# mahaarbo/casclik

Measured on AMD Instinct MI355X. Metric: CLIK steps/sec (whole node), 7-DoF 3-task priority stack, batch 16384, higher is better.
Workload: dtype f64

## Files before the change

casclik_amd/csrc/clik_pinv_team.hpp:

```cpp
#pragma once
#include "clik_pinv_static.hpp"

namespace clik {


constexpr int TEAM_WAVES = 4;
constexpr int TEAM_INST = TEAM_WAVES * WAVE / TEAM;

template <int CTRL>
__device__ __forceinline__ double quad_perm_f64(const double x)
{
    int lo = __double2loint(x), hi = __double2hiint(x);
    lo = __builtin_amdgcn_mov_dpp(lo, CTRL, 0xf, 0xf, true);
    hi = __builtin_amdgcn_mov_dpp(hi, CTRL, 0xf, 0xf, true);
    return __hiloint2double(hi, lo);
}
constexpr int QUAD_LANE0 = 0x00;

template <const ShapeDesc& SD>
inline size_t team_lds_bytes(bool values = false)
{
    if (values) return 0;
    return ((size_t)StaticLayout<SD>::IMG_DOUBLES + (size_t)(SD.n + (SD.n_y > 0 ? SD.n_y : 0)) * TEAM_INST) * sizeof(double);
}

#ifndef CLIK_RESIDENT_PIPELINE
#define CLIK_RESIDENT_PIPELINE 1
#endif

struct RoleConsts {
    double beta, hsel, nsolo, cax, cx2, lam0, kap, hp;
};
__device__ __forceinline__ RoleConsts role_consts_computed(const int r, const double lam)
{
    const double one_lam = 1.0 + lam;
    const bool hi = (r & 2) != 0, solo = (r == 0) || (r == 3);
    RoleConsts rc;
    rc.beta = (r == 1) ? 0.5 * lam : ((r == 2) ? one_lam : lam);
    rc.hsel = solo ? 1.0 : 0.0;
    rc.nsolo = solo ? 0.0 : 1.0;
    rc.cax = hi ? one_lam : 1.0;
    rc.cx2 = hi ? 1.0 : 0.0;
    rc.lam0 = (r == 0) ? lam : 0.0;
    rc.kap = hi ? 1.0 / one_lam : 1.0;
    rc.hp = hi ? 1.0 : 0.0;
    return rc;
}
struct RoleTable {
    double v[TEAM][8];
};
constexpr RoleTable role_table(const double lam)
{
    const double one_lam = 1.0 + lam;
    return RoleTable{{{lam, 1.0, 0.0, 1.0, 0.0, lam, 1.0, 0.0},
                      {0.5 * lam, 0.0, 1.0, 1.0, 0.0, 0.0, 1.0, 0.0},
                      {one_lam, 0.0, 1.0, one_lam, 1.0, 0.0, 1.0 / one_lam, 1.0},
                      {lam, 1.0, 0.0, one_lam, 1.0, 0.0, 1.0 / one_lam, 1.0}}};
}
template <class IMGV>
inline __constant__ RoleTable kRoleTable = role_table(IMGV::value.lam);
#ifndef CLIK_ROLE_TABLE
#define CLIK_ROLE_TABLE 1
#endif
template <class IMGV>
__device__ __forceinline__ RoleConsts role_consts_loaded(const int r)
{
#if !CLIK_ROLE_TABLE
    return role_consts_computed(r, IMGV::value.lam);
#endif
    typedef double d2 __attribute__((ext_vector_type(2)));
    const d2* p = reinterpret_cast<const d2*>(&kRoleTable<IMGV>.v[r][0]);
    const d2 a = p[0], b = p[1], c = p[2], d = p[3];
    return RoleConsts{a.x, a.y, b.x, b.y, c.x, c.y, d.x, d.y};
}

struct NoMidTick {
    __device__ __forceinline__ void operator()(const double) const {}
};
template <const ShapeDesc& SD, class MID = NoMidTick>
__device__ __forceinline__ void team_tick(const Img<SD>* __restrict__ Slds, const TickArgs& tk,
                                          const double (&z)[SD.n], const double* ysl, const double a0, const double a1,
                                          const int r, const int inst, const RoleConsts& rc, const SinCosK& sck,
                                          double (&v)[SD.n], bool& in_tc, MID&& mid = MID())
{
    constexpr int N = SD.n, M = SD.m[1], M0 = SD.m[0], M2 = SD.m[2];
    constexpr int NT = M * (M + 1) / 2;
    TaskCache<SD> tc;
    CLIK_PHASE("sincos");
    {
        double sns[N], css[N];
        if constexpr (SD.uses_fk != 0) {
            double sn0, cs0, sn1, cs1;
            sincos_fast(a0, sn0, cs0, sck);
            sincos_fast(a1, sn1, cs1, sck);
            const bool huge = (fabs(a0) > kSinCosFastMax) | (fabs(a1) > kSinCosFastMax);
            if (__builtin_expect(__ballot(huge) != 0ull, 0)) {
                if (fabs(a0) > kSinCosFastMax) { const SinCos sc = sincos_slow(a0); sn0 = sc.s; cs0 = sc.c; }
                if (fabs(a1) > kSinCosFastMax) { const SinCos sc = sincos_slow(a1); sn1 = sc.s; cs1 = sc.c; }
            }
            CLIK_PHASE("sincos_exchange");
            static_for<0, N>([&](auto jc) __attribute__((always_inline)) {
                constexpr int j = decltype(jc)::value;
                if constexpr (shape_state_type(SD, j) == CLIK_JOINT_REVOLUTE) {
                    constexpr int CTRL = (j / 2) * 0x55;
                    sns[j] = quad_perm_f64<CTRL>((j & 1) ? sn1 : sn0);
                    css[j] = quad_perm_f64<CTRL>((j & 1) ? cs1 : cs0);
                } else {
                    sns[j] = css[j] = 0.0;
                }
            });
        }
        const Img<SD> Sfk = *Slds;
        __builtin_amdgcn_sched_barrier(0);
        CLIK_PHASE("fk");
        Kin<N> K;
        if constexpr (SD.uses_fk != 0) {
            forward_kinematics_sc<SD>(&Sfk, z, sns, css, K);
            if constexpr (SD.quat_src != 0) orientation_feature_s<SD>(&Sfk, ysl, inst, K);
        }
        CLIK_PHASE("task_rows");
        cache_task<SD, 0>(&Sfk, tk, K, z, ysl, inst, tc);
    }

    const Img<SD> Sb = *Slds;
    __builtin_amdgcn_sched_barrier(0);
    CLIK_PHASE("desired");
    const Img<SD>* __restrict__ S = &Sb;
    const double lam = S->lam;
    const double one_lam = 1.0 + lam;

    double des1[M], w2[N];
    {
        double e[M], Jt[M], ke[M];
        task_values<SD, 1>(S, tk, tc, z, ysl, inst, e, Jt);
        gain_apply_s<M, SD.gain_matrix[1] != 0>(S->tasks[1], e, ke);
#pragma unroll
        for (int i = 0; i < M; ++i) des1[i] = SD.feedforward != 0 ? -ke[i] - Jt[i] : -ke[i];
    }
    {
        double e[M2], Jt[M2], ke[M2];
        task_values<SD, 2>(S, tk, tc, z, ysl, inst, e, Jt);
        gain_apply_s<M2, SD.gain_matrix[2] != 0>(S->tasks[2], e, ke);
#pragma unroll
        for (int j = 0; j < N; ++j) w2[j] = 0.0;
        const double* Pm = S->cpinv[2];
        static_for<0, M2>([&](auto ic) __attribute__((always_inline)) {
            constexpr int i = decltype(ic)::value;
            constexpr int col = SD.ucol[2][i] - 1;
            const double d = SD.feedforward != 0 ? -ke[i] - Jt[i] : -ke[i];
            w2[col] = Pm[col * CLIK_MAX_M + i] * d;
        });
    }
    double e0[M0], Jt0[M0];
    task_values<SD, 0>(S, tk, tc, z, ysl, inst, e0, Jt0);
    double sact[N], p0[N];
    static_for<0, M0>([&](auto ic) __attribute__((always_inline)) {
        constexpr int i = decltype(ic)::value;
        constexpr int col = SD.ucol[0][i] - 1;
        sact[col] = ((e0[i] - S->tasks[0].set_max[i] > 0.0) | (e0[i] - S->tasks[0].set_min[i] < 0.0)) ? 1.0 : 0.0;
        p0[col] = S->cpinv[0][col * CLIK_MAX_M + i];
    });

    CLIK_PHASE("gram");
    double Gm[NT];
#pragma unroll
    for (int i = 0; i < M; ++i)
#pragma unroll
        for (int k = 0; k <= i; ++k) {
            double acc = 0.0;
#pragma unroll
            for (int j = 0; j < N; ++j) acc = fma(jac<SD, 1>(S, tc, i, j), jac<SD, 1>(S, tc, k, j), acc);
            Gm[tri(i, k)] = acc;
        }

    if constexpr (!std::is_same<std::decay_t<MID>, NoMidTick>::value) {
        mid(Gm[0]);
    }
    CLIK_PHASE("role_rhs");
    double X[N], rhs[M];
#pragma unroll
    for (int j = 0; j < N; ++j) X[j] = w2[j] * fma(-rc.cx2, sact[j], rc.cax);
#pragma unroll
    for (int i = 0; i < M; ++i) {
        double sacc = 0.0;
#pragma unroll
        for (int j = 0; j < N; ++j) sacc = fma(jac<SD, 1>(S, tc, i, j), X[j], sacc);
        rhs[i] = fma(rc.nsolo, sacc, rc.hsel * des1[i]);
    }
    double A[NT], rd[M], s2[M];
#pragma unroll
    for (int i = 0; i < M; ++i)
#pragma unroll
        for (int k = 0; k <= i; ++k) A[tri(i, k)] = (i == k) ? Gm[tri(i, k)] + rc.beta : Gm[tri(i, k)];
    CLIK_PHASE("factor");
    ldl_factor_s<M>(A, rd);
    CLIK_PHASE("solve1");
    ldl_solve_s<M>(A, rd, rhs);
    CLIK_PHASE("solve2");
#pragma unroll
    for (int i = 0; i < M; ++i) s2[i] = rhs[i];
    ldl_solve_s<M>(A, rd, s2);
#pragma unroll
    for (int i = 0; i < M; ++i) rhs[i] = fma(rc.lam0, s2[i], rhs[i]);
    CLIK_PHASE("jt_product");
    double g[N];
#pragma unroll
    for (int j = 0; j < N; ++j) {
        double sacc = 0.0;
#pragma unroll
        for (int i = 0; i < M; ++i) sacc = fma(jac<SD, 1>(S, tc, i, j), rhs[i], sacc);
        g[j] = sacc;
    }

    
    CLIK_PHASE("meet");
#pragma unroll
    for (int j = 0; j < N; ++j) {
        const double other = quad_perm_f64<0xB1>(g[j]);
        const double nmul = fma(-p0[j] * rc.hp, sact[j], 1.0);
        v[j] = fma(g[j], nmul, rc.kap * (X[j] - other));
    }
    CLIK_PHASE("cone");
    {
        const clik_task& t = S->tasks[0];
        double le[M0], ue[M0];
#pragma unroll
        for (int i = 0; i < M0; ++i) {
            le[i] = e0[i] - t.set_min[i];
            ue[i] = e0[i] - t.set_max[i];
        }
        double le_min = le[0], ue_max = ue[0];
#pragma unroll
        for (int i = 1; i < M0; ++i) {
            le_min = fmin(le_min, le[i]);
            ue_max = fmax(ue_max, ue[i]);
        }
        const bool outside = (le_min < 1e-12) | (ue_max > 1e-12);
        in_tc = true;
        if (__builtin_amdgcn_ballot_w64(outside) != 0ull) {
            double od = 0.0, nde = 0.0, nout = 0.0, ndiff = 0.0;
            static_for<0, M0>([&](auto ic) __attribute__((always_inline)) {
                constexpr int i = decltype(ic)::value;
                constexpr int col = SD.ucol[0][i] - 1;
                const double de = Jt0[i] + v[col];
                const double hl = half_sign(le[i]), hu = half_sign(ue[i]);
                ndiff += fabs(hl - hu);
                const double out = hl + hu;
                od = fma(out, de, od);
                nde = fma(de, de, nde);
                nout = fma(out, out, nout);
            });
            const bool corner = ndiff == 0.0;
            bool going_in = od < 0.0;
            if (__builtin_amdgcn_ballot_w64(corner & outside) != 0ull) {
                const double dists = (sqrt(nde) + 1e-10) * sqrt(nout);
                const bool steep = (od < 0.0) & (fabs(od) / dists < 0.70710678118654757);
                going_in = corner ? steep : going_in;
            }
            in_tc = !outside | going_in;
        }
    }
    CLIK_PHASE_END();
}

template <int K>
struct RawImage {
    unsigned long long w[K];
};

template <const ShapeDesc& SD, class IMGV = void>
__global__ __launch_bounds__(TEAM_WAVES * WAVE) void pinv_solve_static_team_kernel(
    const void* __restrict__ img_g, const double* __restrict__ q, const double* __restrict__ y,
    double* __restrict__ dq, int32_t* __restrict__ mode_out, const long long B, const TickArgs tk)
{
    static_assert(shape_team_ok(SD), "shape outside the team kernel's family");
    constexpr bool VALUES = !std::is_void<IMGV>::value;
    extern __shared__ double lds[];
    constexpr int N = SD.n, M = SD.m[1], M0 = SD.m[0], M2 = SD.m[2], NY = SD.n_y > 0 ? SD.n_y : 0;
    constexpr int NT = M * (M + 1) / 2;
    constexpr int NTHREADS = TEAM_WAVES * WAVE;
    const int tid = threadIdx.x;
    const int wave = __builtin_amdgcn_readfirstlane(tid >> 6);
    const int r = tid & (TEAM - 1);
    const int inst = tid >> 2;
    const long long b0 = (long long)blockIdx.x * TEAM_INST;
    const long long left = B - b0;
    const int rows_valid = left < TEAM_INST ? (int)left : TEAM_INST;
    double* zs = lds + (VALUES ? 0 : StaticLayout<SD>::IMG_DOUBLES);
    double* ys = zs + N * TEAM_INST;
    typedef double d2 __attribute__((ext_vector_type(2)));
    CLIK_STAMP_W(0, 0);
    CLIK_BODY_BEGIN();
    CLIK_PHASE("rows_in");
    const unsigned uinst = (unsigned)blockIdx.x * (unsigned)TEAM_INST + (unsigned)inst;
    const unsigned ulast = (unsigned)B - 1u;
    const unsigned urow = uinst < ulast ? uinst : ulast;
    const long long binst = (long long)urow;
    double zdir[N], ydir[NY > 0 ? NY : 1];
    RoleConsts rc;
    const int j0 = 2 * r < N ? 2 * r : N - 1, j1 = 2 * r + 1 < N ? 2 * r + 1 : N - 1;
    double a0 = 0.0, a1 = 0.0;
    const SinCosK sck = sincos_consts();
    __builtin_amdgcn_sched_barrier(0);
    if constexpr (VALUES) {
        const unsigned qoff = __umul24(urow, (unsigned)(N * sizeof(double)));
        a0 = *reinterpret_cast<const double*>(reinterpret_cast<const char*>(q) + (qoff + (unsigned)j0 * 8u));
        a1 = *reinterpret_cast<const double*>(reinterpret_cast<const char*>(q) + (qoff + (unsigned)j1 * 8u));
        __builtin_amdgcn_sched_barrier(0);
        const double* __restrict__ qrow = reinterpret_cast<const double*>(reinterpret_cast<const char*>(q) + qoff);
#pragma unroll
        for (int j = 0; j < N; ++j) zdir[j] = qrow[j];
        __builtin_amdgcn_sched_barrier(0);
        if constexpr (NY > 0) {
            const double* __restrict__ yrow = reinterpret_cast<const double*>(reinterpret_cast<const char*>(y) + __umul24(urow, (unsigned)(NY * sizeof(double))));
#pragma unroll
            for (int k = 0; k < NY; ++k) ydir[k] = yrow[k];
        }
        __builtin_amdgcn_sched_barrier(0);
        rc = role_consts_loaded<IMGV>(r);
        __builtin_amdgcn_sched_barrier(0);
    }
    if constexpr (!VALUES) {
        constexpr int CH = VALUES ? 0 : StaticLayout<SD>::IMG_CHUNKS;
        constexpr int PER = VALUES ? 1 : (CH + TEAM_WAVES - 1) / TEAM_WAVES;
        constexpr int QR = (N * TEAM_INST + NTHREADS - 1) / NTHREADS;
        constexpr int YR = (NY * TEAM_INST + NTHREADS - 1) / NTHREADS;
        const d2* src = (const d2*)img_g;
        d2* dst = (d2*)lds;
        const int lane = tid & (WAVE - 1);
        d2 img[PER];
        if constexpr (!VALUES) {
#pragma unroll
            for (int k = 0; k < PER; ++k) {
                const int ck = k * TEAM_WAVES + wave;
                img[k] = src[(ck < CH ? ck : CH - 1) * WAVE + lane];
            }
        }
        double qv[QR], yv[YR > 0 ? YR : 1];
        const double* qg = q + b0 * N;
        const int qlast = rows_valid * N - 1;
#pragma unroll
        for (int i = 0; i < QR; ++i) {
            const int k = i * NTHREADS + tid;
            qv[i] = qg[k < qlast ? k : qlast];
        }
        if constexpr (NY > 0) {
            const double* yg = y + b0 * NY;
            const int ylast = rows_valid * NY - 1;
#pragma unroll
            for (int i = 0; i < YR; ++i) {
                const int k = i * NTHREADS + tid;
                yv[i] = yg[k < ylast ? k : ylast];
            }
        }
        if constexpr (!VALUES) {
#pragma unroll
            for (int k = 0; k < PER; ++k) {
                const int ck = k * TEAM_WAVES + wave;
                if (ck < CH) dst[ck * WAVE + lane] = img[k];
            }
        }
#pragma unroll
        for (int i = 0; i < QR; ++i) {
            const int k = i * NTHREADS + tid;
            if (k < N * TEAM_INST) zs[k] = qv[i];
        }
        if constexpr (NY > 0) {
#pragma unroll
            for (int i = 0; i < YR; ++i) {
                const int k = i * NTHREADS + tid;
                if (k < NY * TEAM_INST) ys[k] = yv[i];
            }
        }
        __syncthreads();
    }
    CLIK_STAMP_W(0, 1);
    constexpr Img<SD> Sval = []() constexpr { if constexpr (VALUES) return IMGV::value; else return Img<SD>{}; }();
    const Img<SD>* __restrict__ Slds = VALUES ? &Sval : (const Img<SD>*)lds;
    const double* ysl = VALUES ? ydir : ys + inst * NY;
    if constexpr (!VALUES) rc = role_consts_computed(r, Slds->lam);
    double z[N];
#pragma unroll
    for (int j = 0; j < N; ++j) z[j] = VALUES ? zdir[j] : zs[inst * N + j];

    if constexpr (!VALUES) {
        a0 = zs[inst * N + j0];
        a1 = zs[inst * N + j1];
    }
    double v[N];
    bool in_tc;
    team_tick<SD>(Slds, tk, z, ysl, a0, a1, r, inst, rc, sck, v, in_tc);
    CLIK_STAMP_W(0, 6);
    CLIK_PHASE("select_store");
    const bool ok0 = __builtin_amdgcn_mov_dpp((int)in_tc, QUAD_LANE0, 0xf, 0xf, true) != 0;
    if constexpr (VALUES) {
        if (r == (ok0 ? 0 : 3) && uinst <= ulast) {
            double* __restrict__ drow = reinterpret_cast<double*>(reinterpret_cast<char*>(dq) + __umul24(uinst, (unsigned)(N * sizeof(double))));
#pragma unroll
            for (int j = 0; j < N; ++j) drow[j] = v[j];
            if (mode_out != nullptr)
                *reinterpret_cast<int32_t*>(reinterpret_cast<char*>(mode_out) + uinst * 4u) = ok0 ? 0 : 1;
        }
    } else {
        if (r == (ok0 ? 0 : 3)) {
#pragma unroll
            for (int j = 0; j < N; ++j) zs[inst * N + j] = v[j];
            if (mode_out != nullptr && inst < rows_valid) mode_out[b0 + inst] = ok0 ? 0 : 1;
        }
        __syncthreads();
        constexpr int QR = (N * TEAM_INST + NTHREADS - 1) / NTHREADS;
        double* dg = dq + b0 * N;
        const int total = rows_valid * N;
#pragma unroll
        for (int i = 0; i < QR; ++i) {
            const int k = i * NTHREADS + tid;
            if (k < total) dg[k] = zs[k];
        }
    }
    CLIK_STAMP_W(0, 5);
    CLIK_BODY_END();
    CLIK_PHASE_END();
}

template <const ShapeDesc& SD, class IMGV = void, int STAGES = 1>
__global__ __launch_bounds__(TEAM_WAVES * WAVE) void pinv_rollout_static_team_kernel(
    const void* __restrict__ img_g, double* __restrict__ q, const double* __restrict__ y,
    double* __restrict__ dq, int32_t* __restrict__ mode_out, const long long B,
    const double* __restrict__ tterms, const int n_ticks, const double dt, const double max_speed)
{
    static_assert(STAGES == 1 || STAGES == 4, "explicit Euler or classical Runge-Kutta");
    constexpr int stages = STAGES;
    static_assert(shape_team_ok(SD), "shape outside the team kernel's family");
    constexpr bool VALUES = !std::is_void<IMGV>::value;
    extern __shared__ double lds[];
    constexpr int N = SD.n, NY = SD.n_y > 0 ? SD.n_y : 0;
    const int tid = threadIdx.x;
    const int wave = __builtin_amdgcn_readfirstlane(tid >> 6);
    const int r = tid & (TEAM - 1);
    const int inst = tid >> 2;
    const long long b0 = (long long)blockIdx.x * TEAM_INST;
    const bool valid = b0 + inst < B;
    const long long binst = valid ? (b0 + inst) : (B - 1);
    double* ys = lds + (VALUES ? 0 : StaticLayout<SD>::IMG_DOUBLES);
    double z[N], ydir[NY > 0 ? NY : 1];
#pragma unroll
    for (int j = 0; j < N; ++j) z[j] = q[binst * N + j];
    if constexpr (NY > 0) {
#pragma unroll
        for (int k = 0; k < NY; ++k) ydir[k] = y[binst * NY + k];
    }
    if constexpr (!VALUES) {
        typedef double d2 __attribute__((ext_vector_type(2)));
        constexpr int CH = StaticLayout<SD>::IMG_CHUNKS;
        const d2* src = (const d2*)img_g;
        d2* dst = (d2*)lds;
        const int lane = tid & (WAVE - 1);
        for (int ck = wave; ck < CH; ck += TEAM_WAVES) dst[ck * WAVE + lane] = src[ck * WAVE + lane];
        if constexpr (NY > 0) {
#pragma unroll
            for (int k = 0; k < NY; ++k) ys[inst * NY + k] = ydir[k];
        }
        __syncthreads();
    }
    constexpr Img<SD> Sval = []() constexpr { if constexpr (VALUES) return IMGV::value; else return Img<SD>{}; }();
    const Img<SD>* __restrict__ Slds = VALUES ? &Sval : (const Img<SD>*)lds;
    const double* ysl = VALUES ? ydir : ys + inst * NY;
    RoleConsts rc;
    if constexpr (VALUES) rc = role_consts_loaded<IMGV>(r);
    else rc = role_consts_computed(r, Slds->lam);
    const SinCosK sck = sincos_consts();
    const int nts = Slds->n_tslots;
    double vout[N];
    int acc_mode = -1;
#pragma unroll
    for (int j = 0; j < N; ++j) vout[j] = 0.0;
    const double vmax = max_speed > 0.0 ? max_speed : 1.7976931348623157e308;
    auto accepted = [&](const double (&v)[N], const bool ok0, double (&d)[N]) __attribute__((always_inline)) {
#pragma unroll
        for (int j = 0; j < N; ++j) d[j] = quad_perm_f64<0x00>(v[j]);
        if (__builtin_amdgcn_ballot_w64(!ok0) != 0ull) {
            if (!ok0) {
#pragma unroll
                for (int j = 0; j < N; ++j) d[j] = quad_perm_f64<0xFF>(v[j]);
            }
        }
#pragma unroll
        for (int j = 0; j < N; ++j) d[j] = fmax(fmin(d[j], vmax), -vmax);
    };
    auto sincos_args = [&](const double (&zz)[N], double& a0, double& a1) __attribute__((always_inline)) {
        a0 = zz[N - 1];
        a1 = zz[N - 1];
        static_for<0, TEAM>([&](auto kc) __attribute__((always_inline)) {
            constexpr int k = decltype(kc)::value;
            if constexpr (2 * k < N) a0 = (r == k) ? zz[2 * k] : a0;
            if constexpr (2 * k + 1 < N) a1 = (r == k) ? zz[2 * k + 1] : a1;
        });
    };
#pragma unroll 1
    for (int tick = 0; tick < n_ticks; ++tick) {
        if constexpr (STAGES == 1) {
            asm volatile("" ::: "memory");
            const TickArgs& tk = *reinterpret_cast<const TickArgs*>(tterms + (size_t)tick * 2 * nts);
            double a0, a1;
            sincos_args(z, a0, a1);
            double v[N];
            bool in_tc;
            team_tick<SD>(Slds, tk, z, ysl, a0, a1, r, inst, rc, sck, v, in_tc);
            const bool ok0 = __builtin_amdgcn_mov_dpp((int)in_tc, QUAD_LANE0, 0xf, 0xf, true) != 0;
            accepted(v, ok0, vout);
#pragma unroll
            for (int j = 0; j < N; ++j) z[j] = fma(vout[j], dt, z[j]);
            acc_mode = ok0 ? 0 : 1;
        } else {
        double z0[N], ks[N];
        int mode0 = -1;
#pragma unroll
        for (int j = 0; j < N; ++j) {
            z0[j] = z[j];
            ks[j] = 0.0;
        }
#pragma unroll 1
        for (int st = 0; st < stages; ++st) {
            asm volatile("" ::: "memory");
            const TickArgs& tk = *reinterpret_cast<const TickArgs*>(tterms + ((size_t)tick * stages + st) * 2 * nts);
            double a0, a1;
            sincos_args(z, a0, a1);
            double v[N], d[N];
            bool in_tc;
            team_tick<SD>(Slds, tk, z, ysl, a0, a1, r, inst, rc, sck, v, in_tc);
            const bool ok0 = __builtin_amdgcn_mov_dpp((int)in_tc, QUAD_LANE0, 0xf, 0xf, true) != 0;
            accepted(v, ok0, d);
            const double wgt = (st == 0 || st == 3) ? 1.0 : 2.0;
            const double cnext = (st == 2) ? dt : 0.5 * dt;
#pragma unroll
            for (int j = 0; j < N; ++j) {
                ks[j] = fma(wgt, d[j], ks[j]);
                z[j] = fma(d[j], cnext, z0[j]);
            }
            mode0 = (st == 0) ? (ok0 ? 0 : 1) : mode0;
        }
#pragma unroll
        for (int j = 0; j < N; ++j) {
            vout[j] = ks[j] * (1.0 / 6.0);
            z[j] = fma(vout[j], dt, z0[j]);
        }
        acc_mode = mode0;
        }
    }
    if (r == 0 && valid) {
#pragma unroll
        for (int j = 0; j < N; ++j) {
            q[(b0 + inst) * N + j] = z[j];
            dq[(b0 + inst) * N + j] = vout[j];
        }
        if (mode_out != nullptr) mode_out[b0 + inst] = acc_mode;
    }
}

struct ResidentTicket {
    unsigned in_seq, p0[15];
    unsigned ring_depth, p1a;
    double integrate_dt, max_speed;
    unsigned p1[10];
    unsigned stop, p2[15];
    unsigned waves, ticks_done, p3[14];
};
static_assert(sizeof(ResidentTicket) == 256, "clik_ticket layout (include/clik.h)");

__device__ __forceinline__ unsigned long long realtime_100mhz()
{
    unsigned long long t;
    asm volatile("s_memrealtime %0\n\ts_waitcnt lgkmcnt(0)" : "=s"(t)::"memory");
    return t;
}

template <int NE>
struct RowStage {
    static constexpr int BLOCK = 16 * NE * 8;
    static constexpr int PIECES = (BLOCK + 1023) / 1024;
    static constexpr int DOUBLES = NE > 0 ? PIECES * 128 : 0;
};
template <int NE>
__device__ __forceinline__ int stage_rows(const double* base, const long long row0, const long long total_rows,
                                          double* lds, const int lane, const bool al16)
{
    constexpr int BLOCK = RowStage<NE>::BLOCK;
    long long r0 = row0 < total_rows - 16 ? row0 : total_rows - 16;
    r0 = r0 > 0 ? r0 : 0;
    const char* src = reinterpret_cast<const char*>(base) + r0 * (NE * 8);
    const long long room = (total_rows - r0) * (NE * 8);
    if (al16 && room >= 16) {
#pragma unroll
        for (int p = 0; p < RowStage<NE>::PIECES; ++p) {
            int off = p * 1024 + lane * 16;
            off = off < BLOCK - 16 ? off : BLOCK - 16;
            off = off < room - 16 ? off : (int)(room - 16);
            __builtin_amdgcn_global_load_lds((const __attribute__((address_space(1))) void*)(src + off),
                                             (__attribute__((address_space(3))) void*)(lds + p * 128), 16, 0, 17);
        }
    } else {
#pragma unroll
        for (int p = 0; p < 4 * RowStage<NE>::PIECES; ++p) {
            int off = p * 256 + lane * 4;
            off = off < BLOCK - 4 ? off : BLOCK - 4;
            off = off < room - 4 ? off : (int)(room - 4);
            __builtin_amdgcn_global_load_lds((const __attribute__((address_space(1))) void*)(src + off),
                                             (__attribute__((address_space(3))) void*)(lds + p * 32), 4, 0, 17);
        }
    }
    return (int)(row0 - r0);
}
__device__ __forceinline__ int stage_row(const int i, const int shift) { return (i + shift) < 15 ? (i + shift) : 15; }

struct ResidentWave {
    ResidentTicket* ticket;
    unsigned* done;
    unsigned long long polls, max_polls;
    unsigned seen, slot;
    bool leave, lane0, first;

    __device__ __forceinline__ void init(ResidentTicket* t, unsigned* d, const unsigned long long budget, const int n_ticks,
                                         const unsigned wave_slot, const unsigned n_waves, const int tid)
    {
        ticket = t;
        done = d;
        polls = 0;
        max_polls = budget;
        seen = 0u;
        slot = wave_slot;
        leave = false;
        lane0 = (tid & (WAVE - 1)) == 0;
        first = wave_slot == 0u && tid == 0;
        if (first) {
            ticket->waves = n_waves;
            ticket->p3[0] = (unsigned)budget;
            ticket->p3[1] = (unsigned)(budget >> 32);
            ticket->p3[2] = (unsigned)n_ticks;
        }
    }
    __device__ __forceinline__ void poll_for(const unsigned want)
    {
#pragma unroll 1
        for (;;) {
            seen = __hip_atomic_load(&ticket->in_seq, __ATOMIC_RELAXED, __HIP_MEMORY_SCOPE_SYSTEM);
            if (seen >= want) {
                __atomic_signal_fence(__ATOMIC_ACQUIRE);
                return;
            }
            if (__hip_atomic_load(&ticket->stop, __ATOMIC_RELAXED, __HIP_MEMORY_SCOPE_SYSTEM) != 0u) {
                leave = true;
                return;
            }
            if (++polls > max_polls) {
                __hip_atomic_store(&ticket->stop, 2u, __ATOMIC_RELAXED, __HIP_MEMORY_SCOPE_SYSTEM);
                if (lane0) {
                    ticket->p3[3] = (unsigned)polls;
                    ticket->p3[4] = slot;
                }
                leave = true;
                return;
            }
            __builtin_amdgcn_s_sleep(1);
        }
    }
    __device__ __forceinline__ void peek() { seen = __hip_atomic_load(&ticket->in_seq, __ATOMIC_RELAXED, __HIP_MEMORY_SCOPE_SYSTEM); }
    __device__ __forceinline__ unsigned look() const { return __hip_atomic_load(&ticket->in_seq, __ATOMIC_RELAXED, __HIP_MEMORY_SCOPE_SYSTEM); }
    __device__ __forceinline__ void publish_done(const int k)
    {
        asm volatile("s_waitcnt vmcnt(0)" ::: "memory");
        if (lane0) __hip_atomic_store(done + slot, (unsigned)k, __ATOMIC_RELAXED, __HIP_MEMORY_SCOPE_SYSTEM);
        if (first) ticket->ticks_done = (unsigned)k;
    }
    __device__ __forceinline__ long long ring_depth() const
    {
        const unsigned raw = __hip_atomic_load(&ticket->ring_depth, __ATOMIC_RELAXED, __HIP_MEMORY_SCOPE_SYSTEM);
        return raw > 1u ? (long long)raw : 1ll;
    }
};

template <const ShapeDesc& SD, class IMGV, bool INTEGRATE = false>
__global__ __launch_bounds__(TEAM_WAVES * WAVE) void pinv_resident_team_kernel(
    const double* q, const double* y, double* dq, int32_t* mode_out, const long long B, const TickArgs tk,
    ResidentTicket* ticket, unsigned* done, const int n_ticks, const unsigned long long max_polls)
{
    static_assert(shape_team_ok(SD), "shape outside the team kernel's family");
    static_assert(!std::is_void<IMGV>::value, "resident ticks: value-specialised instantiation only");
    constexpr int N = SD.n, NY = SD.n_y > 0 ? SD.n_y : 0;
    const int tid = threadIdx.x;
    const int r = tid & (TEAM - 1);
    const int inst = tid >> 2;
    const long long b0 = (long long)blockIdx.x * TEAM_INST;
    const bool valid = b0 + inst < B;
    const long long binst = valid ? (b0 + inst) : (B - 1);
    constexpr Img<SD> Sval = IMGV::value;
    CLIK_PHASE("res_setup");
    const RoleConsts rc = role_consts_loaded<IMGV>(r);
    const SinCosK sck = sincos_consts();
    unsigned long long polls = 0;
    if (blockIdx.x == 0 && tid == 0) {
        ticket->waves = gridDim.x * TEAM_WAVES;
        ticket->p3[0] = (unsigned)max_polls;
        ticket->p3[1] = (unsigned)(max_polls >> 32);
        ticket->p3[2] = (unsigned)n_ticks;
    }
    double zn[N], yn[NY > 0 ? NY : 1];
    bool have_next = false, leave = false;
    unsigned seen = 0u;
    auto poll_for = [&](const unsigned want) __attribute__((always_inline)) {
#pragma unroll 1
        for (;;) {
            seen = __hip_atomic_load(&ticket->in_seq, __ATOMIC_RELAXED, __HIP_MEMORY_SCOPE_SYSTEM);
            if (seen >= want) {
                __atomic_signal_fence(__ATOMIC_ACQUIRE);
                return;
            }
            if (__hip_atomic_load(&ticket->stop, __ATOMIC_RELAXED, __HIP_MEMORY_SCOPE_SYSTEM) != 0u) {
                leave = true;
                return;
            }
            if (++polls > max_polls) {
                __hip_atomic_store(&ticket->stop, 2u, __ATOMIC_RELAXED, __HIP_MEMORY_SCOPE_SYSTEM);
                if ((tid & (WAVE - 1)) == 0) {
                    ticket->p3[3] = (unsigned)polls;
                    ticket->p3[4] = blockIdx.x * TEAM_WAVES + (tid >> 6);
                }
                leave = true;
                return;
            }
            __builtin_amdgcn_s_sleep(1);
        }
    };
    const unsigned ring_raw = __hip_atomic_load(&ticket->ring_depth, __ATOMIC_RELAXED, __HIP_MEMORY_SCOPE_SYSTEM);
    const long long ring = ring_raw > 1u ? (long long)ring_raw : 1ll;
    const double step_dt = INTEGRATE ? ticket->integrate_dt : 0.0, step_clamp = INTEGRATE ? ticket->max_speed : 0.0;
    constexpr bool integrate = INTEGRATE;
    double zstate[INTEGRATE ? N : 1];
#pragma unroll
    for (int j = 0; j < (INTEGRATE ? N : 1); ++j) zstate[j] = 0.0;
    constexpr int RQ = (N + 2 * TEAM - 1) / (2 * TEAM);
    using SQ = RowStage<N>;
    using SY = RowStage<NY>;
    __shared__ double stage[TEAM_WAVES][SQ::DOUBLES + SY::DOUBLES + 1];
    const int wv = tid >> 6, lane = tid & (WAVE - 1), iw = inst & 15;
    double* const zs = &stage[wv][0];
    double* const ys = &stage[wv][SQ::DOUBLES];
    const long long total_rows = ring * B;
    const bool al16 = (((unsigned long long)(uintptr_t)q | (unsigned long long)(uintptr_t)y) & 15ull) == 0ull
                      && ((B * N) & 1ll) == 0ll && ((B * NY) & 1ll) == 0ll;
    int shift_q = 0, shift_y = 0;
    auto request_rows = [&](const int k) __attribute__((always_inline)) {
        const long long row0 = ((long long)((k - 1) % (int)ring)) * B + b0 + 16 * wv;
        asm volatile("s_waitcnt lgkmcnt(0)" ::: "memory");
        if (!integrate || k == 1) shift_q = stage_rows<N>(q, row0, total_rows, zs, lane, al16);
        if constexpr (NY > 0) shift_y = stage_rows<NY>(y, row0, total_rows, ys, lane, al16);
    };
    auto read_rows = [&]() __attribute__((always_inline)) {
        const int iq = stage_row(iw, shift_q) * N;
#pragma unroll
        for (int j = 0; j < N; ++j) zn[j] = zs[iq + j];
        if constexpr (NY > 0) {
            const int iy = stage_row(iw, shift_y) * NY;
#pragma unroll
            for (int j = 0; j < NY; ++j) yn[j] = ys[iy + j];
        }
    };
    auto publish_done = [&](const int k) __attribute__((always_inline)) {
// ... 146 lines not shown
```

casclik_amd/csrc/clik_pinv_kernels.hpp:

```cpp
#pragma once
#include "clik_device.hpp"
#include "clik_pinv_static.hpp"
#include "clik_pinv_select.hpp"

namespace clik {

struct Stack {
    int      r;
    bool     gram;
    uint32_t sbits;
};

template <int N>
__device__ __forceinline__ void stack_push(Stack& st, double* wk, int lane, const int n, const int cap,
                                           const double lam, const double (&J)[N][N], const int m,
                                           const uint32_t srow, const int times)
{
    constexpr int NT = N * (N + 1) / 2;
    if (!st.gram && st.r + times * m <= cap) {
#pragma unroll
        for (int rep = 0; rep < 2; ++rep) {
            if (rep < times) {
                const int r0 = st.r;
#pragma unroll
// ... 988 lines not shown
            pinv_tick_static<SD>(&Sreg, tk, z, ys + lane * SD.n_y, lane, valid, vout, acc_mode);
#pragma unroll
            for (int j = 0; j < N; ++j) {
                double d = vout[j];
                if (j < NQ && max_speed > 0.0) d = fmax(fmin(d, max_speed), -max_speed);
                vout[j] = d;
                z[j] = fma(d, dt, z[j]);
            }
        }
    } else {
        double* z0s = ys + SD.n_y * WAVE;
        double* kss = z0s + N * WAVE;
#pragma unroll 1
        for (int tick = 0; tick < n_ticks; ++tick) {
            int mode0 = -1;
#pragma unroll
            for (int j = 0; j < N; ++j) {
                z0s[j * WAVE + lane] = z[j];
                kss[j * WAVE + lane] = 0.0;
            }
#pragma unroll 1
            for (int st = 0; st < 4; ++st) {
                asm volatile("" ::: "memory");
                const TickArgs& tk = *reinterpret_cast<const TickArgs*>(tterms + ((size_t)tick * 4 + st) * 2 * nts);
                pinv_tick_static<SD>(S, tk, z, ys + lane * SD.n_y, lane, valid, vout, acc_mode);
                const double wgt = (st == 0 || st == 3) ? 1.0 : 2.0;
                const double cnext = (st == 2) ? dt : 0.5 * dt;
#pragma unroll
                for (int j = 0; j < N; ++j) {
                    double d = vout[j];
                    if (j < NQ && max_speed > 0.0) d = fmax(fmin(d, max_speed), -max_speed);
                    kss[j * WAVE + lane] = fma(wgt, d, kss[j * WAVE + lane]);
                    z[j] = fma(d, cnext, z0s[j * WAVE + lane]);
                }
                mode0 = (st == 0) ? acc_mode : mode0;
            }
#pragma unroll
            for (int j = 0; j < N; ++j) {
                vout[j] = kss[j * WAVE + lane] * (1.0 / 6.0);
                z[j] = fma(vout[j], dt, z0s[j * WAVE + lane]);
            }
            acc_mode = mode0;
        }
    }
    __syncthreads();
    state_to_lds<NQ, NX>(z, zs, xs, lane);
    __syncthreads();
    rows_from_lds<NQ>(q + b0 * NQ, rows_valid, zs, lane);
    if constexpr (NX > 0) rows_from_lds<NX>(x + b0 * NX, rows_valid, xs, lane);
    __syncthreads();
    state_to_lds<NQ, NX>(vout, zs, xs, lane);
    __syncthreads();
    rows_from_lds<NQ>(dq + b0 * NQ, rows_valid, zs, lane);
    if constexpr (NX > 0) rows_from_lds<NX>(dx + b0 * NX, rows_valid, xs, lane);
    if (mode_out != nullptr && valid) mode_out[b0 + lane] = acc_mode;
}

}
#include "clik_pinv_team.hpp"
namespace clik {

#ifndef CLIK_DEFER_INPUT_ROWS
#define CLIK_DEFER_INPUT_ROWS 1
#endif
typedef hipError_t (*solve_fn)(const LaunchArgs&, const TickArgs&, long long, const double*, const double*,
                               const double*, double*, double*, int32_t*, hipStream_t);
typedef hipError_t (*rollout_fn)(const LaunchArgs&, const double*, int, double, double, long long, double*,
                                 const double*, double*, int32_t*, hipStream_t);

template <int N, class SH>
inline hipError_t launch_solve(const LaunchArgs& a, const TickArgs& tk, long long B, const double* q,
                               const double* x, const double* y, double* dq, double* dx, int32_t* mode,
                               hipStream_t stream)
{
    if (a.t_inst != nullptr) return hipErrorNotSupported;
    const unsigned grid = (unsigned)((B + WAVE - 1) / WAVE);
    const size_t shmem = (size_t)pinv_lds_slots(N, a.ny) * WAVE * sizeof(double);
    hipLaunchKernelGGL((pinv_solve_kernel<N, SH>), dim3(grid), dim3(WAVE), shmem, stream, a.dS, *a.warm, tk, B, q,
                       x, y, dq, dx, mode);
    return hipGetLastError();
}

template <int N, class SH>
inline hipError_t launch_rollout(const LaunchArgs& a, const double* d_tterms, int n_ticks, double dt,
                                 double max_speed, long long B, double* q, const double* y, double* dq,
                                 int32_t* mode, hipStream_t stream)
{
    const unsigned grid = (unsigned)((B + WAVE - 1) / WAVE);
    const size_t shmem = (size_t)pinv_lds_slots(N, a.ny) * WAVE * sizeof(double);
    hipLaunchKernelGGL((pinv_rollout_kernel<N, SH>), dim3(grid), dim3(WAVE), shmem, stream, a.dS, *a.warm,
                       d_tterms, n_ticks, dt, max_speed, B, q, y, dq, mode);
    return hipGetLastError();
}

template <const ShapeDesc& SD>
inline size_t static_lds_bytes(int ny)
{
    return ((size_t)StaticLayout<SD>::IMG_DOUBLES + (size_t)(SD.n + ny) * WAVE) * sizeof(double);
}

template <const ShapeDesc& SD>
inline hipError_t launch_solve_static(const LaunchArgs& a, const TickArgs& tk, long long B, const double* q,
                                      const double* x, const double* y, double* dq, double* dx, int32_t* mode,
                                      hipStream_t stream)
{
    const unsigned grid = (unsigned)((B + WAVE - 1) / WAVE);
    if (a.t_inst != nullptr) {
        hipLaunchKernelGGL((pinv_solve_static_pt_kernel<SD>), dim3(grid), dim3(WAVE), static_lds_bytes<SD>(a.ny), stream,
                           a.dImg, q, y, dq, mode, B, x, dx, a.t_inst);
        return hipGetLastError();
    }
    PinvPolicy p = a.policy;
    p.values_attached = false;
    switch (pinv_select(SD, p, B, PinvOp::tick)) {
    case PinvVariant::team4:
        if constexpr (shape_team_ok(SD)) {
            hipLaunchKernelGGL((pinv_solve_static_team_kernel<SD>), dim3(grid), dim3(TEAM_WAVES * WAVE),
                               team_lds_bytes<SD>(), stream, a.dImg, q, y, dq, mode, B, tk);
            return hipGetLastError();
        }
        break;
    case PinvVariant::mp2:
    case PinvVariant::mp4:
        if constexpr ((StaticLayout<SD>::n_sets == 1 || StaticLayout<SD>::n_sets == 2) && SD.n_x == 0) {
            constexpr int NM = 1 << StaticLayout<SD>::n_sets;
            const size_t shmem = static_lds_bytes<SD>(a.ny) + (size_t)(NM - 1) * (SD.n + 1) * WAVE * sizeof(double);
            hipLaunchKernelGGL((pinv_solve_static_mp_kernel<SD>), dim3(grid), dim3(NM * WAVE), shmem, stream,
                               a.dImg, q, y, dq, mode, B, tk);
            return hipGetLastError();
        }
        break;
    case PinvVariant::lane_occ2:
#ifdef CLIK_LARGE_BATCH_VARIANT
        hipLaunchKernelGGL((pinv_solve_static_occ2_kernel<SD>), dim3(grid), dim3(WAVE), static_lds_bytes<SD>(a.ny), stream,
                           a.dImg, q, y, dq, mode, B, x, dx, tk);
        return hipGetLastError();
#else
        break;
#endif
    default:
        break;
    }
    hipLaunchKernelGGL((pinv_solve_static_kernel<SD>), dim3(grid), dim3(WAVE), static_lds_bytes<SD>(a.ny), stream,
                       a.dImg, q, y, dq, mode, B, x, dx, tk);
    return hipGetLastError();
}

template <const ShapeDesc& SD, class IMGV>
inline hipError_t launch_solve_team_values(const LaunchArgs& a, const TickArgs& tk, long long B, const double* q,
                                           const double* y, double* dq, int32_t* mode, hipStream_t stream)
{
    static_assert(shape_team_ok(SD), "value-specialised kernels exist for the team family only");
    const unsigned grid = (unsigned)((B + TEAM_INST - 1) / TEAM_INST);
    hipLaunchKernelGGL((pinv_solve_static_team_kernel<SD, IMGV>), dim3(grid), dim3(TEAM_WAVES * WAVE),
                       team_lds_bytes<SD>(true), stream, nullptr, q, y, dq, mode, B, tk);
    (void)a;
    return hipGetLastError();
}

constexpr unsigned long long kResidentIntegrateBit = 1ull << 63;
template <const ShapeDesc& SD, class IMGV>
inline hipError_t launch_resident_quad_values(const TickArgs& tk, long long B, const double* q, const double* y, double* dq,
                                              int32_t* mode, void* ticket, unsigned* done, int n_ticks,
                                              unsigned long long timeout_ticks, hipStream_t stream);

template <const ShapeDesc& SD, class IMGV>
inline hipError_t launch_resident_team_values(const TickArgs& tk, long long B, const double* q, const double* y,
                                              double* dq, int32_t* mode, void* ticket, unsigned* done, int n_ticks,
                                              unsigned long long timeout_ticks, hipStream_t stream)
{
    if constexpr (shape_team_ok(SD)) {
        const unsigned grid = (unsigned)((B + TEAM_INST - 1) / TEAM_INST);
        const unsigned long long budget = timeout_ticks & ~kResidentIntegrateBit;
        {
            static int max_blocks[2] = {-1, -1};
            const int which = (timeout_ticks & kResidentIntegrateBit) ? 1 : 0;
            if (max_blocks[which] < 0) {
                int per_cu = 0, dev = 0, cus = 0;
                hipError_t oe = which
                    ? hipOccupancyMaxActiveBlocksPerMultiprocessor(&per_cu, pinv_resident_team_kernel<SD, IMGV, true>,
                                                                   TEAM_WAVES * WAVE, 0)
                    : hipOccupancyMaxActiveBlocksPerMultiprocessor(&per_cu, pinv_resident_team_kernel<SD, IMGV, false>,
                                                                   TEAM_WAVES * WAVE, 0);
                if (oe == hipSuccess) oe = hipGetDevice(&dev);
                if (oe == hipSuccess) oe = hipDeviceGetAttribute(&cus, hipDeviceAttributeMultiprocessorCount, dev);
                if (oe != hipSuccess) return oe;
                max_blocks[which] = per_cu >= 1 ? cus : 0;
            }
            if ((long long)grid > (long long)max_blocks[which]) return hipErrorNotSupported;
        }
        if (timeout_ticks & kResidentIntegrateBit)
            hipLaunchKernelGGL((pinv_resident_team_kernel<SD, IMGV, true>), dim3(grid), dim3(TEAM_WAVES * WAVE), 0, stream,
                               q, y, dq, mode, B, tk, (ResidentTicket*)ticket, done, n_ticks, budget);
        else
            hipLaunchKernelGGL((pinv_resident_team_kernel<SD, IMGV, false>), dim3(grid), dim3(TEAM_WAVES * WAVE), 0, stream,
                               q, y, dq, mode, B, tk, (ResidentTicket*)ticket, done, n_ticks, budget);
        return hipGetLastError();
    } else {
        return launch_resident_quad_values<SD, IMGV>(tk, B, q, y, dq, mode, ticket, done, n_ticks, timeout_ticks, stream);
    }
}

template <const ShapeDesc& SD, class IMGV>
inline hipError_t launch_rollout_team_values(const LaunchArgs& a, const double* d_tterms, int n_ticks, double dt,
                                             double max_speed, long long B, double* q, const double* y, double* dq,
                                             int32_t* mode, hipStream_t stream)
{
    static_assert(shape_team_ok(SD), "value-specialised kernels exist for the team family only");
    const unsigned grid = (unsigned)((B + TEAM_INST - 1) / TEAM_INST);
    if (a.roll_stages == 4)
        hipLaunchKernelGGL((pinv_rollout_static_team_kernel<SD, IMGV, 4>), dim3(grid), dim3(TEAM_WAVES * WAVE),
                           team_rollout_lds_bytes<SD>(true), stream, nullptr, q, y, dq, mode, B, d_tterms, n_ticks, dt, max_speed);
    else
        hipLaunchKernelGGL((pinv_rollout_static_team_kernel<SD, IMGV, 1>), dim3(grid), dim3(TEAM_WAVES * WAVE),
                           team_rollout_lds_bytes<SD>(true), stream, nullptr, q, y, dq, mode, B, d_tterms, n_ticks, dt, max_speed);
    return hipGetLastError();
}

template <const ShapeDesc& SD, class IMGV>
__global__ __launch_bounds__(WAVE) CLIK_OCC_ATTR void pinv_solve_static_values_kernel(
    const double* __restrict__ q, const double* __restrict__ y, double* __restrict__ dq,
    int32_t* __restrict__ mode_out, const long long B, const TickArgs tk)
{
    static_assert(SD.n_x == 0, "value-specialised lane kernel: robot variables only");
    CLIK_BODY_BEGIN();
    constexpr int N = SD.n;
    constexpr Img<SD> Sval = IMGV::value;
    const int lane = threadIdx.x;
    const long long inst = (long long)blockIdx.x * WAVE + lane;
    const bool valid = inst < B;
    const long long row = valid ? inst : B - 1;
    double z[N];
#pragma unroll
    for (int j = 0; j < N; ++j) z[j] = q[row * N + j];
    const double* ys = SD.n_y > 0 ? y + row * SD.n_y : nullptr;
#if CLIK_DEFER_INPUT_ROWS
    double yrow[SD.n_y > 0 ? SD.n_y : 1];
    if constexpr (SD.n_y > 0) {
        double dep = z[0];
        int off = 0;
        asm volatile("" : "+v"(off) : "v"(dep));
        const double* yp = ys + off;
#pragma unroll
        for (int k = 0; k < SD.n_y; ++k) yrow[k] = yp[k];
        __builtin_amdgcn_sched_barrier(0);
        ys = yrow;
    }
#endif
    double vout[N];
    int acc_mode;
    pinv_tick_static<SD>(&Sval, tk, z, ys, lane, valid, vout, acc_mode);
    if (valid) {
#pragma unroll
        for (int j = 0; j < N; ++j) dq[inst * N + j] = vout[j];
        if (mode_out != nullptr) mode_out[inst] = acc_mode;
    }
    CLIK_BODY_END();
}

template <const ShapeDesc& SD, class IMGV>
__global__ __launch_bounds__(WAVE) CLIK_OCC_ATTR void pinv_solve_static_values_quad_kernel(
    const double* __restrict__ q, const double* __restrict__ y, double* __restrict__ dq,
    int32_t* __restrict__ mode_out, const long long B, const TickArgs tk)
{
    static_assert(SD.n_x == 0, "value-specialised kernels: robot variables only");
    CLIK_BODY_BEGIN();
    constexpr int N = SD.n;
    constexpr Img<SD> Sval = IMGV::value;
    const int tid = threadIdx.x;
    const int r = tid & (TEAM - 1);
    CLIK_PHASE("rows_in");
    const SinCosK sck = sincos_consts();
    __builtin_amdgcn_sched_barrier(0);
    const unsigned inst = (unsigned)blockIdx.x * (unsigned)(WAVE / TEAM) + ((unsigned)tid >> 2);
    const unsigned last = (unsigned)B - 1u;
    const bool valid = inst <= last;
    const unsigned row = inst < last ? inst : last;
    const unsigned qoff = __umul24(row, (unsigned)(N * sizeof(double)));
    const double* __restrict__ qrow = reinterpret_cast<const double*>(reinterpret_cast<const char*>(q) + qoff);
    const int j0 = 2 * r < N ? 2 * r : N - 1, j1 = 2 * r + 1 < N ? 2 * r + 1 : N - 1;
    const double a0 = *reinterpret_cast<const double*>(reinterpret_cast<const char*>(q) + (qoff + (unsigned)j0 * 8u));
    const double a1 = *reinterpret_cast<const double*>(reinterpret_cast<const char*>(q) + (qoff + (unsigned)j1 * 8u));
    __builtin_amdgcn_sched_barrier(0);
    double z[N];
#pragma unroll
    for (int j = 0; j < N; ++j) z[j] = qrow[j];
    constexpr int NYQ = SD.n_y > 0 ? SD.n_y : 0;
    double ydir[NYQ > 0 ? NYQ : 1];
    if constexpr (NYQ > 0) {
        const double* __restrict__ yrow =
            reinterpret_cast<const double*>(reinterpret_cast<const char*>(y) + __umul24(row, (unsigned)(NYQ * sizeof(double))));
#pragma unroll
        for (int k = 0; k < NYQ; ++k) ydir[k] = yrow[k];
    }
    asm volatile("" ::: "memory");
    const double* ys = NYQ > 0 ? ydir : nullptr;
    CLIK_PHASE("sincos");
    double sn0, cs0, sn1, cs1;
    sincos_fast(a0, sn0, cs0, sck);
    sincos_fast(a1, sn1, cs1, sck);
    const bool huge = (fabs(a0) > kSinCosFastMax) | (fabs(a1) > kSinCosFastMax);
    if (__builtin_expect(__builtin_amdgcn_ballot_w64(huge) != 0ull, 0)) {
        if (fabs(a0) > kSinCosFastMax) { const SinCos sc = sincos_slow(a0); sn0 = sc.s; cs0 = sc.c; }
        if (fabs(a1) > kSinCosFastMax) { const SinCos sc = sincos_slow(a1); sn1 = sc.s; cs1 = sc.c; }
    }
    CLIK_PHASE("sincos_exchange");
    double sns[N], css[N];
    static_for<0, N>([&](auto jc) __attribute__((always_inline)) {
        constexpr int j = decltype(jc)::value;
// ... 350 lines not shown
```

Baseline: 4.068 billion.

## Stage q/y rows through LDS via direct global-to-LDS loads in values team kernel

In the values-specialized team kernel, per-thread strided loads of each instance's q and y rows are replaced by coalesced wave-wide global_load_lds copies of 16 rows into a per-wave shared-memory stage, followed by LDS reads. Role constants are now computed from the lambda value while the loads are in flight, instead of being loaded. The staging helper moves earlier in the file and is templated on index type and cache-policy bits. This aims to cut uncoalesced global traffic for small rows, at the cost of extra static LDS, a full vmcnt wait, and 32-bit index arithmetic that assumes B fits in int.

```diff
diff --git a/casclik_amd/csrc/clik_pinv_team.hpp b/casclik_amd/csrc/clik_pinv_team.hpp
--- a/casclik_amd/csrc/clik_pinv_team.hpp
+++ b/casclik_amd/csrc/clik_pinv_team.hpp
@@ -262,6 +262,44 @@
     }
     CLIK_PHASE_END();
 }
+
+template <int NE>
+struct RowStage {
+    static constexpr int BLOCK = 16 * NE * 8;
+    static constexpr int PIECES = (BLOCK + 1023) / 1024;
+    static constexpr int DOUBLES = NE > 0 ? PIECES * 128 : 0;
+};
+template <int NE, int AUX = 17, class I = long long>
+__device__ __forceinline__ int stage_rows(const double* base, const I row0, const I total_rows,
+                                          double* lds, const int lane, const bool al16)
+{
+    constexpr int BLOCK = RowStage<NE>::BLOCK;
+    I r0 = row0 < total_rows - 16 ? row0 : total_rows - 16;
+    r0 = r0 > 0 ? r0 : 0;
+    const char* src = reinterpret_cast<const char*>(base) + r0 * (NE * 8);
+    const I room = (total_rows - r0) * (NE * 8);
+    if (al16 && room >= 16) {
+#pragma unroll
+        for (int p = 0; p < RowStage<NE>::PIECES; ++p) {
+            int off = p * 1024 + lane * 16;
+            off = off < BLOCK - 16 ? off : BLOCK - 16;
+            off = off < room - 16 ? off : (int)(room - 16);
+            __builtin_amdgcn_global_load_lds((const __attribute__((address_space(1))) void*)(src + off),
+                                             (__attribute__((address_space(3))) void*)(lds + p * 128), 16, 0, AUX);
+        }
+    } else {
+#pragma unroll
+        for (int p = 0; p < 4 * RowStage<NE>::PIECES; ++p) {
+            int off = p * 256 + lane * 4;
+            off = off < BLOCK - 4 ? off : BLOCK - 4;
+            off = off < room - 4 ? off : (int)(room - 4);
+            __builtin_amdgcn_global_load_lds((const __attribute__((address_space(1))) void*)(src + off),
+                                             (__attribute__((address_space(3))) void*)(lds + p * 32), 4, 0, AUX);
+        }
+    }
+    return (int)(row0 - r0);
+}
+__device__ __forceinline__ int stage_row(const int i, const int shift) { return (i + shift) < 15 ? (i + shift) : 15; }
 
 template <int K>
 struct RawImage {
@@ -307,18 +345,29 @@
         a0 = *reinterpret_cast<const double*>(reinterpret_cast<const char*>(q) + (qoff + (unsigned)j0 * 8u));
         a1 = *reinterpret_cast<const double*>(reinterpret_cast<const char*>(q) + (qoff + (unsigned)j1 * 8u));
         __builtin_amdgcn_sched_barrier(0);
-        const double* __restrict__ qrow = reinterpret_cast<const double*>(reinterpret_cast<const char*>(q) + qoff);
-#pragma unroll
-        for (int j = 0; j < N; ++j) zdir[j] = qrow[j];
+        using SQ = RowStage<N>;
+        using SY = RowStage<NY>;
+        __shared__ double stage[TEAM_WAVES][SQ::DOUBLES + SY::DOUBLES];
+        const int lane = tid & (WAVE - 1), iw = inst & 15;
+        double* const zst = &stage[wave][0];
+        double* const yst = &stage[wave][SQ::DOUBLES];
+        const int row0 = (int)blockIdx.x * TEAM_INST + 16 * wave;
+        const bool al16 = (((unsigned long long)(uintptr_t)q | (unsigned long long)(uintptr_t)y) & 15ull) == 0ull
+                          && (((unsigned)B * (unsigned)N) & 1u) == 0u && (((unsigned)B * (unsigned)NY) & 1u) == 0u;
+        const int shift_q = stage_rows<N, 17, int>(q, row0, (int)B, zst, lane, al16);
+        int shift_y = 0;
+        if constexpr (NY > 0) shift_y = stage_rows<NY, 17, int>(y, row0, (int)B, yst, lane, al16);
         __builtin_amdgcn_sched_barrier(0);
+        rc = role_consts_computed(r, IMGV::value.lam);
+        asm volatile("s_waitcnt vmcnt(0)" ::: "memory");
+        const int iq = stage_row(iw, shift_q) * N;
+#pragma unroll
+        for (int j = 0; j < N; ++j) zdir[j] = zst[iq + j];
         if constexpr (NY > 0) {
-            const double* __restrict__ yrow = reinterpret_cast<const double*>(reinterpret_cast<const char*>(y) + __umul24(urow, (unsigned)(NY * sizeof(double))));
-#pragma unroll
-            for (int k = 0; k < NY; ++k) ydir[k] = yrow[k];
-        }
-        __builtin_amdgcn_sched_barrier(0);
-        rc = role_consts_loaded<IMGV>(r);
-        __builtin_amdgcn_sched_barrier(0);
+            const int iy = stage_row(iw, shift_y) * NY;
+#pragma unroll
+            for (int k = 0; k < NY; ++k) ydir[k] = yst[iy + k];
+        }
     }
     if constexpr (!VALUES) {
         constexpr int CH = VALUES ? 0 : StaticLayout<SD>::IMG_CHUNKS;
@@ -574,44 +623,6 @@
     return t;
 }
 
-template <int NE>
-struct RowStage {
-    static constexpr int BLOCK = 16 * NE * 8;
-    static constexpr int PIECES = (BLOCK + 1023) / 1024;
-    static constexpr int DOUBLES = NE > 0 ? PIECES * 128 : 0;
-};
-template <int NE>
-__device__ __forceinline__ int stage_rows(const double* base, const long long row0, const long long total_rows,
-                                          double* lds, const int lane, const bool al16)
-{
-    constexpr int BLOCK = RowStage<NE>::BLOCK;
-    long long r0 = row0 < total_rows - 16 ? row0 : total_rows - 16;
-    r0 = r0 > 0 ? r0 : 0;
-    const char* src = reinterpret_cast<const char*>(base) + r0 * (NE * 8);
-    const long long room = (total_rows - r0) * (NE * 8);
-    if (al16 && room >= 16) {
-#pragma unroll
-        for (int p = 0; p < RowStage<NE>::PIECES; ++p) {
-            int off = p * 1024 + lane * 16;
-            off = off < BLOCK - 16 ? off : BLOCK - 16;
-            off = off < room - 16 ? off : (int)(room - 16);
-            __builtin_amdgcn_global_load_lds((const __attribute__((address_space(1))) void*)(src + off),
-                                             (__attribute__((address_space(3))) void*)(lds + p * 128), 16, 0, 17);
-        }
-    } else {
-#pragma unroll
-        for (int p = 0; p < 4 * RowStage<NE>::PIECES; ++p) {
-            int off = p * 256 + lane * 4;
-            off = off < BLOCK - 4 ? off : BLOCK - 4;
-            off = off < room - 4 ? off : (int)(room - 4);
-            __builtin_amdgcn_global_load_lds((const __attribute__((address_space(1))) void*)(src + off),
-                                             (__attribute__((address_space(3))) void*)(lds + p * 32), 4, 0, 17);
-        }
-    }
-    return (int)(row0 - r0);
-}
-__device__ __forceinline__ int stage_row(const int i, const int shift) { return (i + shift) < 15 ? (i + shift) : 15; }
-
 struct ResidentWave {
     ResidentTicket* ticket;
     unsigned* done;
```

After: 3.930 billion. 0.966x the previous value.

## Add full-batch team solve kernel with direct row loads and stores

Applied to the files above, without the earlier changes.

Adds a specialised team solve kernel for value-specialised shapes whose target width equals the joint count, used when the batch divides evenly into team instances. It skips LDS staging and bounds checks, loads q and y rows straight from global memory using byte offsets computed with 24-bit multiplies and a perm-based piece table, and has one lane per team write the result row and mode directly. It also defers the corner-case norm sums in the cone check to the rare branch and merges two range compares into one fmax. In exchange there is an extra kernel variant to maintain, and the direct per-lane strided global stores may coalesce worse than the old staged LDS copy-out.

```diff
diff --git a/casclik_amd/csrc/clik_pinv_kernels.hpp b/casclik_amd/csrc/clik_pinv_kernels.hpp
--- a/casclik_amd/csrc/clik_pinv_kernels.hpp
+++ b/casclik_amd/csrc/clik_pinv_kernels.hpp
@@ -1164,9 +1164,20 @@
 {
     static_assert(shape_team_ok(SD), "value-specialised kernels exist for the team family only");
     const unsigned grid = (unsigned)((B + TEAM_INST - 1) / TEAM_INST);
+    (void)a;
+    if constexpr (team_full_ok<SD>()) {
+        if (B % TEAM_INST == 0) {
+            if (mode != nullptr)
+                hipLaunchKernelGGL((pinv_solve_team_full_kernel<SD, IMGV, true>), dim3(grid), dim3(TEAM_WAVES * WAVE), 0,
+                                   stream, q, y, dq, mode, tk);
+            else
+                hipLaunchKernelGGL((pinv_solve_team_full_kernel<SD, IMGV, false>), dim3(grid), dim3(TEAM_WAVES * WAVE), 0,
+                                   stream, q, y, dq, nullptr, tk);
+            return hipGetLastError();
+        }
+    }
     hipLaunchKernelGGL((pinv_solve_static_team_kernel<SD, IMGV>), dim3(grid), dim3(TEAM_WAVES * WAVE),
                        team_lds_bytes<SD>(true), stream, nullptr, q, y, dq, mode, B, tk);
-    (void)a;
     return hipGetLastError();
 }
 
diff --git a/casclik_amd/csrc/clik_pinv_team.hpp b/casclik_amd/csrc/clik_pinv_team.hpp
--- a/casclik_amd/csrc/clik_pinv_team.hpp
+++ b/casclik_amd/csrc/clik_pinv_team.hpp
@@ -93,7 +93,7 @@
             double sn0, cs0, sn1, cs1;
             sincos_fast(a0, sn0, cs0, sck);
             sincos_fast(a1, sn1, cs1, sck);
-            const bool huge = (fabs(a0) > kSinCosFastMax) | (fabs(a1) > kSinCosFastMax);
+            const bool huge = fmax(fabs(a0), fabs(a1)) > kSinCosFastMax;
             if (__builtin_expect(__ballot(huge) != 0ull, 0)) {
                 if (fabs(a0) > kSinCosFastMax) { const SinCos sc = sincos_slow(a0); sn0 = sc.s; cs0 = sc.c; }
                 if (fabs(a1) > kSinCosFastMax) { const SinCos sc = sincos_slow(a1); sn1 = sc.s; cs1 = sc.c; }
@@ -103,8 +103,9 @@
                 constexpr int j = decltype(jc)::value;
                 if constexpr (shape_state_type(SD, j) == CLIK_JOINT_REVOLUTE) {
                     constexpr int CTRL = (j / 2) * 0x55;
-                    sns[j] = quad_perm_f64<CTRL>((j & 1) ? sn1 : sn0);
-                    css[j] = quad_perm_f64<CTRL>((j & 1) ? cs1 : cs0);
+                    constexpr bool second = (j & 1) != 0 || ((N & 1) != 0 && j == N - 1);
+                    sns[j] = quad_perm_f64<CTRL>(second ? sn1 : sn0);
+                    css[j] = quad_perm_f64<CTRL>(second ? cs1 : cs0);
                 } else {
                     sns[j] = css[j] = 0.0;
                 }
@@ -238,21 +239,26 @@
         const bool outside = (le_min < 1e-12) | (ue_max > 1e-12);
         in_tc = true;
         if (__builtin_amdgcn_ballot_w64(outside) != 0ull) {
-            double od = 0.0, nde = 0.0, nout = 0.0, ndiff = 0.0;
+            double od = 0.0, ndiff = 0.0;
+            double de[M0], out[M0];
             static_for<0, M0>([&](auto ic) __attribute__((always_inline)) {
                 constexpr int i = decltype(ic)::value;
                 constexpr int col = SD.ucol[0][i] - 1;
-                const double de = Jt0[i] + v[col];
+                de[i] = Jt0[i] + v[col];
                 const double hl = half_sign(le[i]), hu = half_sign(ue[i]);
                 ndiff += fabs(hl - hu);
-                const double out = hl + hu;
-                od = fma(out, de, od);
-                nde = fma(de, de, nde);
-                nout = fma(out, out, nout);
+                out[i] = hl + hu;
+                od = fma(out[i], de[i], od);
             });
             const bool corner = ndiff == 0.0;
             bool going_in = od < 0.0;
             if (__builtin_amdgcn_ballot_w64(corner & outside) != 0ull) {
+                double nde = 0.0, nout = 0.0;
+#pragma unroll
+                for (int i = 0; i < M0; ++i) {
+                    nde = fma(de[i], de[i], nde);
+                    nout = fma(out[i], out[i], nout);
+                }
                 const double dists = (sqrt(nde) + 1e-10) * sqrt(nout);
                 const bool steep = (od < 0.0) & (fabs(od) / dists < 0.70710678118654757);
                 going_in = corner ? steep : going_in;
@@ -422,6 +428,62 @@
     CLIK_PHASE_END();
 }
 
+template <const ShapeDesc& SD>
+constexpr bool team_full_ok() { return SD.n_y == SD.n; }
+
+template <const ShapeDesc& SD, class IMGV, bool MODE>
+__global__ __launch_bounds__(TEAM_WAVES * WAVE) void pinv_solve_team_full_kernel(
+    const double* __restrict__ q, const double* __restrict__ y, double* __restrict__ dq, int32_t* __restrict__ mode_out,
+    const TickArgs tk)
+{
+    static_assert(shape_team_ok(SD), "shape outside the team kernel's family");
+    static_assert(!std::is_void<IMGV>::value && team_full_ok<SD>(), "full-batch form: value-specialised, one row pitch");
+    constexpr int N = SD.n, NY = SD.n_y;
+    CLIK_BODY_BEGIN();
+    CLIK_PHASE("rows_in");
+    const int tid = threadIdx.x;
+    const int r = tid & (TEAM - 1);
+    constexpr unsigned PITCH = (unsigned)(N * sizeof(double));
+    const unsigned roff = __umul24((unsigned)tid >> 2, PITCH) + (unsigned)blockIdx.x * ((unsigned)TEAM_INST * PITCH);
+    static_assert(PITCH >= 16u && PITCH - 16u < 256u, "the piece's offset is a byte of the table");
+    constexpr auto piece = [](unsigned k) constexpr { return 16u * k < PITCH - 16u ? 16u * k : PITCH - 16u; };
+    constexpr unsigned PIECES = piece(0) | piece(1) << 8 | piece(2) << 16 | piece(3) << 24;
+    const unsigned a_in_row = __builtin_amdgcn_perm(0u, PIECES, (unsigned)r);
+    typedef double d2 __attribute__((ext_vector_type(2)));
+    const d2 a01 = *reinterpret_cast<const d2*>(reinterpret_cast<const char*>(q) + (roff + a_in_row));
+    __builtin_amdgcn_sched_barrier(0);
+    double z[N], ydir[NY];
+    const double* __restrict__ qrow = reinterpret_cast<const double*>(reinterpret_cast<const char*>(q) + roff);
+#pragma unroll
+    for (int j = 0; j < N; ++j) z[j] = qrow[j];
+    __builtin_amdgcn_sched_barrier(0);
+    const double* __restrict__ yrow = reinterpret_cast<const double*>(reinterpret_cast<const char*>(y) + roff);
+#pragma unroll
+    for (int k = 0; k < NY; ++k) ydir[k] = yrow[k];
+    __builtin_amdgcn_sched_barrier(0);
+    const RoleConsts rc = role_consts_loaded<IMGV>(r);
+    __builtin_amdgcn_sched_barrier(0);
+    const SinCosK sck = sincos_consts();
+    __builtin_amdgcn_sched_barrier(0);
+    constexpr Img<SD> Sval = IMGV::value;
+    double v[N];
+    bool in_tc;
+    team_tick<SD>(&Sval, tk, z, ydir, a01.x, a01.y, r, tid >> 2, rc, sck, v, in_tc);
+    CLIK_PHASE("select_store");
+    const int ok0 = __builtin_amdgcn_mov_dpp((int)in_tc, QUAD_LANE0, 0xf, 0xf, true);
+    if (r == 3 - 3 * ok0) {
+        double* __restrict__ drow = reinterpret_cast<double*>(reinterpret_cast<char*>(dq) + roff);
+#pragma unroll
+        for (int j = 0; j < N; ++j) drow[j] = v[j];
+        if constexpr (MODE) {
+            const unsigned moff = ((unsigned)tid & ~(unsigned)(TEAM - 1)) + (unsigned)blockIdx.x * ((unsigned)TEAM_INST * 4u);
+            *reinterpret_cast<int32_t*>(reinterpret_cast<char*>(mode_out) + moff) = 1 - ok0;
+        }
+    }
+    CLIK_BODY_END();
+    CLIK_PHASE_END();
+}
+
 template <const ShapeDesc& SD, class IMGV = void, int STAGES = 1>
 __global__ __launch_bounds__(TEAM_WAVES * WAVE) void pinv_rollout_static_team_kernel(
     const void* __restrict__ img_g, double* __restrict__ q, const double* __restrict__ y,
```

Result: no change. 4.057 billion before, 4.048 billion after, median of 2 (-0.2%).
